# RozDavid/UnScene3D

Hardware: AMD Instinct MI355X
Metric: training scenes/sec (Res16UNet34C+Mask3D, 150k voxels) (higher is better)
Workload: dtype f32

## Files before the change

include/usc3d.h:

```cpp
#ifndef USC3D_H
#define USC3D_H

#include <stdint.h>

#ifdef __cplusplus
extern "C" {
#endif

typedef void* usc_stream_t;

enum usc_status {
  USC_OK = 0,
  USC_ERR_ARG = -1,
  USC_ERR_LAUNCH = -2,
  USC_ERR_RANGE = -3
};

const char* usc_last_error(void);
int usc_abi_version(void);
const char* usc_build_info(void);
int usc_device_count(void);


int usc_voxel_floor_f64(const double* xyz, int64_t n, double voxel_size,
// ... 261 lines not shown
                         float* invstd, float* scale, float* shift, void* ws,
                         int64_t ws_bytes, usc_stream_t s);
int usc_bn_apply(const float* x, const float* scale, const float* shift,
                 const float* residual, int32_t relu, float* y, int64_t n,
                 int32_t c, usc_stream_t s);
int usc_bn_backward_dx(const float* x, const float* dy, const float* y_out,
                       const float* mean, const float* invstd,
                       const float* gamma, const float* mean_g,
                       const float* mean_gxhat, float* dx, float* dres,
                       int64_t n, int32_t c, usc_stream_t s);
int64_t usc_bn_tile_max_rows(void);
int64_t usc_bn_plan(int64_t n, int32_t c, int32_t backward);
int usc_bn_tile_ok(int64_t n, int32_t c);
int64_t usc_bn_tile_ws_bytes(int32_t c);
int usc_bn_tile_forward(const float* partial, int32_t G, float* y, int64_t n,
                        int32_t c, const float* gamma, const float* beta,
                        float eps, float momentum, float* running_mean,
                        float* running_var, int64_t* num_batches_tracked,
                        float* mean, float* invstd, float* scale, float* shift,
                        const float* residual, int32_t relu, float* out,
                        void* ws, int64_t ws_bytes, usc_stream_t s);
int usc_bn_tile_backward(const float* partial, int32_t G, int32_t accumulate,
                         float* dout, const float* y, const float* y_out,
                         const float* mean, const float* invstd,
                         const float* gamma, int64_t n, int32_t c,
                         int32_t training, int32_t dbn_accumulate,
                         float* dgamma, float* dbeta, float* dy, float* dres,
                         void* ws, int64_t ws_bytes, usc_stream_t s);
int usc_bn_backward_reduce(const float* x, const float* dy, const float* y_out,
                           const float* mean, const float* invstd, int64_t n,
                           int32_t c, int32_t training, int32_t accumulate, float* dgamma,
                           float* dbeta, float* mean_g, float* mean_gxhat,
                           void* ws, int64_t ws_bytes, usc_stream_t s);
int usc_relu_fwd(const float* x, float* y, int64_t numel, usc_stream_t s);
int usc_relu_bwd(const float* y, const float* dy, float* dx, int64_t numel,
                 usc_stream_t s);

int usc_avgpool_down2(const float* in, int32_t c, const int32_t* nbr2,
                      int64_t n_coarse, float* out, usc_stream_t s);
int usc_avgpool_down2_ex(const float* in, int32_t c, int32_t ld,
                         const int64_t* row_of, const int32_t* nbr2,
                         int64_t n_coarse, float* out, uint8_t* mask_out,
                         usc_stream_t s);

int usc_gather_rows(const float* src, int32_t c, const int64_t* idx, int64_t n,
                    float* out, usc_stream_t s);

int usc_scatter_add_rows(const float* src, int32_t c, const int64_t* idx,
                         int64_t n, float* dst, usc_stream_t s);

int usc_scatter_rows_unique(const float* src, int32_t c, const int64_t* idx,
                            int64_t n, float* dst, usc_stream_t s);
int usc_scatter_rows_unique_add(const float* src, int32_t c, const int64_t* idx,
                                int64_t n, float* dst, usc_stream_t s);

int64_t usc_sample_keys_ws_bytes(int32_t n_scenes, int32_t K, int32_t q);
int usc_sample_keys(const float* feats, int32_t c, const uint8_t* mask, int32_t q, const float* pos, int32_t p,
                    const int64_t* idx, int32_t n_scenes, int32_t K, const int32_t* n_valid, float* out_feats,
                    uint8_t* out_mask, float* out_pos, void* ws, int64_t ws_bytes, usc_stream_t s);

int64_t usc_attn_mask_rows_ws_bytes(int32_t n_scenes, int32_t K, int32_t q, int32_t d);
int usc_attn_mask_rows(const float* in, int32_t ld, int32_t q, int32_t d, const int32_t* const* tabs,
                       const int64_t* n_rows, const int64_t* idx, int32_t n_scenes, int32_t K,
                       const int32_t* n_valid, uint8_t* out_mask, void* ws, int64_t ws_bytes, int32_t skip_fix,
                       usc_stream_t s);

// ... 373 lines not shown
```

unscene3d_amd/_lib.py:

```python
from __future__ import annotations

import ctypes as C
import os

import torch

_HERE = os.path.dirname(os.path.abspath(__file__))
LIB_PATH = os.environ.get("USC3D_LIB") or os.path.join(_HERE, "libusc3d_hip.so")

_p = C.c_void_p
_i32 = C.c_int32
_i64 = C.c_int64
_f64 = C.c_double
_f32 = C.c_float

class KMap(C.Structure):
    _fields_ = [("nbr", _p), ("perm", _p), ("tile_mask", _p), ("pair_in", _p), ("pair_out", _p), ("koff", _p),
                ("n_in", _i64), ("n_out", _i64), ("pair_capacity", _i64), ("K", _i32), ("reserved", _i32)]


class BNDesc(C.Structure):
    _fields_ = [("gamma", _p), ("beta", _p), ("running_mean", _p), ("running_var", _p), ("num_batches_tracked", _p),
                ("eps", _f32), ("momentum", _f32), ("c", _i32), ("training", _i32)]

# ... 71 lines not shown
    "usc_spconv_wgrad_group_max": (_i32, []),
    "usc_spconv_wgrad_grid_limit": (None, [_i32]),
    "usc_spconv_wgrad_group_ok": (C.c_int, [_i32, _i32, _i32, _i32, _i64]),
    "usc_spconv_wgrad_group": (C.c_int, [_i32, _p, _p, _p, _i32, _i32, _i32, _p, _p, _p, _i64, _i32, _p]),
    "usc_spconv_wgrad_table_ws_bytes": (_i64, [_i32, _i32, _i32]),
    "usc_spconv_wgrad_table": (C.c_int, [_p, _i32, _p, _i32, _p, _i32, _i64, _p, _i32, _p, _i64, _p]),
    "usc_set_wgrad_lane": (C.c_int, [_p, _p, _i64, _i64]),
    "usc_wgrad_lane_join": (C.c_int, [_p]),
    "usc_wgrad_lane_hold": (C.c_int, [_i32, _i64, _i64, _p]),
    "usc_wgrad_lane_holding": (_i32, []),
    "usc_launch_stats_begin": (C.c_int, [_p, _i64, _p]),
    "usc_launch_stats_end": (_i64, [_p, _i64]),
    "usc_wall_clock_khz": (_i64, []),
    "usc_conv_ws_bytes": (_i64, [_kp, _i32, _i32, _i32]),
    "usc_unit_ws_bytes": (_i64, [_kp, _i32, _i32, _i32]),
    "usc_conv_forward": (C.c_int, [_kp, _i32, _p, _i32, _p, _i32, _p, _p, _p, _i64, _p]),
    "usc_conv_backward": (C.c_int, [_kp, _i32, _p, _i32, _p, _i32, _p, _p, _i32, _p, _i32, _p, _i64, _p]),
    "usc_bn_eval_stats": (C.c_int, [_p, _p, _p, _p, _f32, _i32, _p, _p, _p, _p, _p]),
    "usc_conv_bn_act_forward": (C.c_int, [_kp, _i32, _p, _i32, _p, _i32, _bp, _p, _i32, _p, _p, _p, _p, _i64, _p]),
    "usc_unit_bf16_ws_bytes": (_i64, [_kp, _i32, _i32, _i32]),
    "usc_conv_bn_act_forward_bf16": (C.c_int, [_kp, _i32, _p, _i32, _p, _i32, _bp, _p, _i32, _p, _p, _p, _p, _i64, _p]),
    "usc_unit_split_ws_bytes": (_i64, [_kp, _i32, _i32, _i32, _i32]),
    "usc_conv_bn_act_forward_split": (C.c_int, [_kp, _i32, _p, _i32, _p, _i32, _i32, _bp, _p, _i32, _p, _p, _p, _p, _i64, _p]),
    "usc_conv_bn_act_backward_split": (C.c_int, [_kp, _i32, _p, _i32, _p, _i32, _i32, _bp, _p, _p, _p, _p, _p, _p, _p, _i32, _p,
                                                 _i32, _p, _p, _i32, _p, _i64, _p]),
    "usc_conv_bn_act_backward": (C.c_int, [_kp, _i32, _p, _i32, _p, _i32, _bp, _p, _p, _p, _p, _p, _p, _p, _i32, _p,
                                           _i32, _p, _p, _i32, _p, _i64, _p]),
    "usc_colstats_ws_bytes": (_i64, [_i64, _i32]),
    "usc_colstats": (C.c_int, [_p, _p, _i64, _i32, _p, _p, _p, _i64, _p]),
    "usc_bn_apply": (C.c_int, [_p, _p, _p, _p, _i32, _p, _i64, _i32, _p]),
    "usc_bn_backward_dx": (C.c_int, [_p, _p, _p, _p, _p, _p, _p, _p, _p, _p, _i64, _i32, _p]),
    "usc_bn_backward_reduce": (C.c_int, [_p, _p, _p, _p, _p, _i64, _i32, _i32, _i32, _p, _p, _p, _p, _p, _i64, _p]),
    "usc_bn_forward_stats": (C.c_int, [_p, _i64, _i32, _p, _p, _f32, _f32, _p, _p, _p, _p, _p, _p, _p, _p, _i64, _p]),
    "usc_relu_fwd": (C.c_int, [_p, _p, _i64, _p]),
    "usc_relu_bwd": (C.c_int, [_p, _p, _p, _i64, _p]),
    "usc_avgpool_down2": (C.c_int, [_p, _i32, _p, _i64, _p, _p]),
    "usc_avgpool_down2_ex": (C.c_int, [_p, _i32, _i32, _p, _p, _i64, _p, _p, _p]),
    "usc_gather_rows": (C.c_int, [_p, _i32, _p, _i64, _p, _p]),
    "usc_scatter_add_rows": (C.c_int, [_p, _i32, _p, _i64, _p, _p]),
    "usc_scatter_rows_unique": (C.c_int, [_p, _i32, _p, _i64, _p, _p]),
    "usc_scatter_rows_unique_add": (C.c_int, [_p, _i32, _p, _i64, _p, _p]),
    "usc_sample_keys_ws_bytes": (_i64, [_i32, _i32, _i32]),
    "usc_sample_keys": (C.c_int, [_p, _i32, _p, _i32, _p, _i32, _p, _i32, _i32, _p, _p, _p, _p, _p, _i64, _p]),
    "usc_attn_mask_rows_ws_bytes": (_i64, [_i32, _i32, _i32, _i32]),
    "usc_attn_mask_rows": (C.c_int, [_p, _i32, _i32, _i32, _p, _p, _p, _i32, _i32, _p, _p, _p, _i64, _i32, _p]),
    "usc_segment_csr_ws_bytes": (_i64, [_i64, _i64]),
    "usc_segment_csr": (C.c_int, [_p, _i64, _i64, _p, _p, _p, _i64, _p]),
    "usc_segment_mean_fwd": (C.c_int, [_p, _i32, _p, _p, _i64, _p, _p]),
    "usc_segment_mean_bwd": (C.c_int, [_p, _i32, _p, _p, _i64, _p, _p]),
    "usc_segment_mean_nonzero": (C.c_int, [_p, _i32, _p, _p, _i64, _p, _p, _p]),
    "usc_segment_max_nonzero": (C.c_int, [_p, _i32, _p, _p, _i64, _p, _p, _p]),
    "usc_ncut_similarity": (C.c_int, [_p, _i64, _i32, _i32, _p, _p, _p]),
    "usc_ncut_similarity_masked": (C.c_int, [_p, _p, _i64, _i32, _i32, _p, _p, _p]),
    "usc_ncut_normalize_mat": (C.c_int, [_p, _i64, _p, _i64, _p]),
    "usc_ncut_binarize": (C.c_int, [_p, _p, _i64, _f32, _f64, _p, _p, _p, _p]),
    "usc_ncut_fiedler_ws_bytes": (_i64, [_i64]),
    "usc_ncut_fiedler": (C.c_int, [_p, _p, _i64, _f64, _p, _p, _p, _i64, _p]),
    "usc_ncut_fiedler_ex": (C.c_int, [_p, _p, _i64, _f64, _p, _p, _p, _i64, _p, _i32]),
    "usc_ncut_fiedler_plan": (_i32, [_i64, _i32, _i32]),
    "usc_knn1": (C.c_int, [_p, _i64, _p, _i64, _p, _p, _p]),
    "usc_knn1_grid_ws_bytes": (_i64, [_i64, _p]),
    "usc_knn1_grid": (C.c_int, [_p, _i64, _p, _i64, _p, _f64, _p, _p, _p, _p, _i64, _p]),
    "usc_knn_hybrid_grid_ws_bytes": (_i64, [_i64, _p]),
    "usc_knn_hybrid_grid": (C.c_int, [_p, _i64, _p, _i64, _f32, _i32, _p, _f64, _p, _p, _p, _p, _i64, _p]),
    "usc_normals_pca": (C.c_int, [_p, _i64, _p, _i64, _p, _p, _i32, _p, _p]),
    "usc_cc_eps_init": (C.c_int, [_p, _i64, _p]),
# ... 148 lines not shown
```

unscene3d_amd/csrc/rows.hip:

```cpp
#include <math.h>
#include <stdlib.h>

#include "common.h"
#include "scan.h"

namespace usc {

void launch_group_reduce(const float* partial, int G, int64_t numel4, int cout, const float* bias, int accumulate,
                         float* out, hipStream_t st);

enum StatMode { STAT_XY = 0, STAT_BN_BWD = 1 };

struct StatArgs {
  const float* x;
  const float* y;
  const float* y_out;
  const float* mean;
  const float* invstd;
  int64_t n;
  int c;
};

constexpr int kStatMaxBlocks = 1024;
constexpr int kStatUnroll = 4;

template <int VEC, int MODE>
__global__ __launch_bounds__(256) void colstats_kernel(StatArgs a, double* __restrict__ partial) {
  extern __shared__ double sh[];
  const int c = a.c;
  const int CT = c / VEC;
  const int RP = 256 / CT;
  const int rl = threadIdx.x / CT, cg = threadIdx.x - rl * CT;
  const bool active = rl < RP;
  double s1[VEC], s2[VEC];
#pragma unroll
  for (int v = 0; v < VEC; ++v) s1[v] = s2[v] = 0.0;
  float mu[VEC], is[VEC];
  if (MODE == STAT_BN_BWD && active) {
#pragma unroll
    for (int v = 0; v < VEC; ++v) {
      mu[v] = a.mean[cg * VEC + v];
      is[v] = a.invstd[cg * VEC + v];
    }
  }
  if (active) {
    const int64_t stride = (int64_t)gridDim.x * RP;
    for (int64_t r0 = (int64_t)blockIdx.x * RP + rl; r0 < a.n; r0 += stride * kStatUnroll) {
      float xv[kStatUnroll][VEC], yv[kStatUnroll][VEC], ov[kStatUnroll][VEC];
#pragma unroll
      for (int u = 0; u < kStatUnroll; ++u) {
        const int64_t r = r0 + u * stride;
        if (r < a.n) {
          const int64_t off = r * c + cg * VEC;
          if (VEC == 4) {
            float4 t = *reinterpret_cast<const float4*>(a.x + off);
            xv[u][0] = t.x; xv[u][1] = t.y; xv[u][2] = t.z; xv[u][3] = t.w;
            if (a.y) {
              float4 w = *reinterpret_cast<const float4*>(a.y + off);
              yv[u][0] = w.x; yv[u][1] = w.y; yv[u][2] = w.z; yv[u][3] = w.w;
            }
            if (MODE == STAT_BN_BWD && a.y_out) {
              float4 w = *reinterpret_cast<const float4*>(a.y_out + off);
              ov[u][0] = w.x; ov[u][1] = w.y; ov[u][2] = w.z; ov[u][3] = w.w;
            }
          } else {
            xv[u][0] = a.x[off];
            if (a.y) yv[u][0] = a.y[off];
            if (MODE == STAT_BN_BWD && a.y_out) ov[u][0] = a.y_out[off];
          }
        }
      }
#pragma unroll
      for (int u = 0; u < kStatUnroll; ++u) {
        if (r0 + u * stride < a.n) {
#pragma unroll
          for (int v = 0; v < VEC; ++v) {
            if (MODE == STAT_XY) {
              s1[v] += (double)xv[u][v];
              s2[v] += (double)xv[u][v] * (double)(a.y ? yv[u][v] : xv[u][v]);
            } else {
              float g = yv[u][v];
              if (a.y_out && !(ov[u][v] > 0.f)) g = 0.f;
              const float xhat = (xv[u][v] - mu[v]) * is[v];
              s1[v] += (double)g;
              s2[v] += (double)g * (double)xhat;
            }
          }
        }
      }
    }
#pragma unroll
    for (int v = 0; v < VEC; ++v) {
      sh[((int64_t)rl * c + cg * VEC + v) * 2 + 0] = s1[v];
      sh[((int64_t)rl * c + cg * VEC + v) * 2 + 1] = s2[v];
    }
  }
  __syncthreads();
  for (int ch = threadIdx.x; ch < c; ch += 256) {
    double t1 = 0.0, t2 = 0.0;
    for (int r = 0; r < RP; ++r) {
      t1 += sh[((int64_t)r * c + ch) * 2 + 0];
// ... 157 lines not shown
    }
  }
}

__global__ void bn_eval_stats_kernel(const float* __restrict__ gamma, const float* __restrict__ beta,
                                     const float* __restrict__ rmean, const float* __restrict__ rvar, float eps, int c,
                                     float* __restrict__ mean, float* __restrict__ invstd, float* __restrict__ scale,
                                     float* __restrict__ shift) {
  const int ch = blockIdx.x * blockDim.x + threadIdx.x;
  if (ch >= c) return;
  const float is = 1.f / sqrtf(rvar[ch] + eps);
  const float sc = gamma[ch] * is;
  mean[ch] = rmean[ch];
  invstd[ch] = is;
  scale[ch] = sc;
  shift[ch] = beta[ch] - rmean[ch] * sc;
}

static int colstats_vec(int c) {
  if (c < 1 || c > 1024) return 0;
  const int vec = (c % 4 == 0 && c / 4 <= 256) ? 4 : 1;
  return c / vec <= 256 ? vec : 0;
}
static int colstats_blocks(int64_t n, int c, int vec) {
  const int CT = c / vec, RP = 256 / CT;
  int64_t b = ceil_div(n, (int64_t)RP * 4 * kStatUnroll);
  if (b > kStatMaxBlocks) b = kStatMaxBlocks;
  if (b < 1) b = 1;
  return (int)b;
}

template <int MODE>
static int launch_colstats_partials(const StatArgs& a, void* ws, int64_t ws_bytes, hipStream_t st, const char* name,
                                    int* nblocks_out) {
  const int c = a.c;
  const int vec = colstats_vec(c);
  USC_REQUIRE(vec > 0, "%s: unsupported channel count %d", name, c);
  const int nb = colstats_blocks(a.n, c, vec);
  USC_REQUIRE(ws_bytes >= (int64_t)nb * 2 * c * 8, "%s: workspace too small", name);
  const int RP = 256 / (c / vec);
  const size_t lds = (size_t)RP * c * 2 * sizeof(double);
  double* partial = (double*)ws;
  if (vec == 4)
    hipLaunchKernelGGL((colstats_kernel<4, MODE>), dim3(nb), dim3(256), lds, st, a, partial);
  else
    hipLaunchKernelGGL((colstats_kernel<1, MODE>), dim3(nb), dim3(256), lds, st, a, partial);
  *nblocks_out = nb;
  return USC_OK;
}

constexpr int kSampleRows = 16;
constexpr int kSampleMaxQ = 256;
constexpr int kSampleMaxScenes = 16;
struct SampleArgs {
  const float* feats; const unsigned char* mask; const float* pos; const int64_t* idx;
  float* out_feats; unsigned char* out_mask; float* out_pos; unsigned char* part;
  int c, q, p, K, nblk, qs;
  int n_valid[kSampleMaxScenes];
};

template <int NQ>
__global__ __launch_bounds__(256) void sample_keys_kernel(SampleArgs a) {
  __shared__ unsigned char acc[4][128 * NQ];
  const int lane = threadIdx.x & 63, wave = threadIdx.x >> 6;
  const int b = blockIdx.y, k0 = blockIdx.x * kSampleRows + wave * 4;
  const int c4 = a.c >> 2, p4 = a.p >> 2;
  const int nvalid = a.n_valid[b];
  const bool has_pos = a.pos != nullptr;
  int64_t src[4];
#pragma unroll
  for (int r = 0; r < 4; ++r) {
    const int k = k0 + r < a.K ? k0 + r : a.K - 1;
    src[r] = a.idx[(int64_t)b * a.K + k];
  }
  float4 f0[4], f1[4], q0[4], q1[4];
  unsigned char ma[4], mb[4], mc[NQ > 1 ? 4 : 1], md[NQ > 1 ? 4 : 1];
  const bool fa = lane < c4, fb = lane + 64 < c4, pa = has_pos && lane < p4, pb = has_pos && lane + 64 < p4;
  const bool qa = lane < a.q, qb = lane + 64 < a.q, qc = NQ > 1 && lane + 128 < a.q, qd = NQ > 1 && lane + 192 < a.q;
#pragma unroll
// ... 906 lines not shown
    const float4 mx = *reinterpret_cast<const float4*>(tile_sh + c + ch0);
    const float ga0 = a.gamma[ch0], ga1 = a.gamma[ch0 + 1], ga2 = a.gamma[ch0 + 2], ga3 = a.gamma[ch0 + 3];
    float4 o;
    o.x = ga0 * is.x * (gv.x - mg.x - (xv.x - mu.x) * is.x * mx.x);
    o.y = ga1 * is.y * (gv.y - mg.y - (xv.y - mu.y) * is.y * mx.y);
    o.z = ga2 * is.z * (gv.z - mg.z - (xv.z - mu.z) * is.z * mx.z);
    o.w = ga3 * is.w * (gv.w - mg.w - (xv.w - mu.w) * is.w * mx.w);
    *reinterpret_cast<float4*>(a.dx + e) = o;
  }
}

struct BnTileGeom { int tr, ntiles, ncb; };
static BnTileGeom bn_tile_geom(int64_t n, int c) {
  BnTileGeom g;
  const int64_t per = ceil_div(n, (int64_t)kBnTileMaxTiles);
  g.tr = (int)(ceil_div(per, (int64_t)kBnTileRowLanes) * kBnTileRowLanes);
  g.ntiles = (int)ceil_div(n, (int64_t)g.tr);
  g.ncb = c / 32;
  return g;
}
static int bn_apply_grid(int64_t nvec) {
  int64_t g = ceil_div(nvec, (int64_t)256 * 2);
  if (g > 1024) g = 1024;
  if (g < 1) g = 1;
  return (int)g;
}

static bool tile_form_on() {
  static const bool on = usc_bn_tile_max_rows() > 0;
  return on;
}
bool tile_rows_ok(int64_t n, int c) { return tile_form_on() && n <= usc_bn_tile_max_rows() && usc_bn_tile_ok(n, c); }

}

using namespace usc;

extern "C" {

int64_t usc_bn_plan(int64_t n, int32_t c, int32_t backward) {
  USC_REQUIRE(n >= 1 && c >= 1, "usc_bn_plan: bad sizes");
  int64_t code = 0;
  if (bn_small_ok(n, c, backward != 0)) {
    code = 1 | ((int64_t)bn_small_remap(c / 4) << 2);
  } else if (const int vec = colstats_vec(c)) {
    code = 2 | ((int64_t)vec << 3) | ((int64_t)colstats_blocks(n, c, vec) << 8);
  }
  if (usc_bn_tile_ok(n, c)) {
    const BnTileGeom g = bn_tile_geom(n, c);
    code |= ((int64_t)1 << 20) | ((int64_t)g.ntiles << 24) | ((int64_t)g.tr << 32);
  }
  if (tile_rows_ok(n, c)) code |= (int64_t)1 << 21;
  return code;
}

int64_t usc_colstats_ws_bytes(int64_t n, int32_t c) { (void)n; return (int64_t)kStatMaxBlocks * 2 * c * 8; }

int usc_colstats(const float* x, const float* y, int64_t n, int32_t c, double* sum1, double* sum2, void* ws,
                 int64_t ws_bytes, usc_stream_t s) {
  USC_REQUIRE(x && sum1 && sum2 && ws && n >= 0, "usc_colstats: bad argument");
  StatArgs a{x, y, nullptr, nullptr, nullptr, n, (int)c};
  int nb = 0;
  int rc = launch_colstats_partials<STAT_XY>(a, ws, ws_bytes, as_stream(s), "usc_colstats", &nb);
  if (rc) return rc;
  hipLaunchKernelGGL(colstats_final_kernel, dim3((unsigned)c), dim3(64), 0, as_stream(s), (const double*)ws, nb, (int)c,
                     sum1, sum2);
// ... 21 lines not shown
  USC_CHECK_LAUNCH("usc_bn_forward_stats");
  return USC_OK;
}

int usc_bn_eval_stats(const float* gamma, const float* beta, const float* running_mean, const float* running_var, float eps,
                      int32_t c, float* mean, float* invstd, float* scale, float* shift, usc_stream_t s) {
  USC_REQUIRE(gamma && beta && running_mean && running_var && mean && invstd && scale && shift && c >= 1,
              "usc_bn_eval_stats: bad argument");
  hipLaunchKernelGGL(bn_eval_stats_kernel, dim3((unsigned)ceil_div(c, 256)), dim3(256), 0, as_stream(s), gamma, beta,
                     running_mean, running_var, eps, (int)c, mean, invstd, scale, shift);
  USC_CHECK_LAUNCH("usc_bn_eval_stats");
  return USC_OK;
}

int usc_bn_backward_reduce(const float* x, const float* dy, const float* y_out, const float* mean, const float* invstd,
                           int64_t n, int32_t c, int32_t training, int32_t accumulate, float* dgamma, float* dbeta,
                           float* mean_g, float* mean_gxhat, void* ws, int64_t ws_bytes, usc_stream_t s) {
  USC_REQUIRE(x && dy && mean && invstd && dgamma && dbeta && mean_g && mean_gxhat && ws && n >= 1,
              "usc_bn_backward_reduce: bad argument");
  StatArgs a{x, dy, y_out, mean, invstd, n, (int)c};
  BnBwdOut o{dgamma, dbeta, mean_g, mean_gxhat, n, (int)training, (int)accumulate};
  if (bn_small_ok(n, c, true)) {
    hipLaunchKernelGGL((bn_small_kernel<STAT_BN_BWD, BnBwdOut>), dim3((unsigned)(c / 4)), dim3(256), 0, as_stream(s), a, o);
    USC_CHECK_LAUNCH("usc_bn_backward_reduce");
    return USC_OK;
  }
  int nb = 0;
  int rc = launch_colstats_partials<STAT_BN_BWD>(a, ws, ws_bytes, as_stream(s), "usc_bn_backward_reduce", &nb);
  if (rc) return rc;
  hipLaunchKernelGGL(bn_bwd_finalize_kernel, dim3((unsigned)c), dim3(64), 0, as_stream(s), (const double*)ws, nb, (int)c, o);
  USC_CHECK_LAUNCH("usc_bn_backward_reduce");
  return USC_OK;
}

int usc_bn_apply(const float* x, const float* scale, const float* shift, const float* residual, int32_t relu, float* y,
                 int64_t n, int32_t c, usc_stream_t s) {
  USC_REQUIRE(n >= 0 && c >= 1, "usc_bn_apply: bad sizes");
  if (n == 0) return USC_OK;
  USC_REQUIRE(x && scale && shift && y, "usc_bn_apply: null pointer");
  const int64_t numel = n * c;
  if (c % 4 == 0)
    hipLaunchKernelGGL((bn_apply_kernel<4>), dim3(stream_grid(numel / 4, 256)), dim3(256), 0, as_stream(s), x, scale,
                       shift, residual, (int)relu, y, numel / 4, (int)c);
  else
    hipLaunchKernelGGL((bn_apply_kernel<1>), dim3(stream_grid(numel, 256)), dim3(256), 0, as_stream(s), x, scale,
                       shift, residual, (int)relu, y, numel, (int)c);
  USC_CHECK_LAUNCH("usc_bn_apply");
  return USC_OK;
}

int usc_bn_backward_dx(const float* x, const float* dy, const float* y_out, const float* mean, const float* invstd,
                       const float* gamma, const float* mean_g, const float* mean_gxhat, float* dx, float* dres,
                       int64_t n, int32_t c, usc_stream_t s) {
  USC_REQUIRE(n >= 0 && c >= 1, "usc_bn_backward_dx: bad sizes");
  if (n == 0) return USC_OK;
  USC_REQUIRE(x && dy && mean && invstd && gamma && mean_g && mean_gxhat && dx, "usc_bn_backward_dx: null pointer");
  const int64_t numel = n * c;
  if (c % 4 == 0)
    hipLaunchKernelGGL((bn_bwd_dx_kernel<4>), dim3(stream_grid(numel / 4, 256)), dim3(256), 0, as_stream(s), x, dy,
                       y_out, mean, invstd, gamma, mean_g, mean_gxhat, dx, dres, numel / 4, (int)c);
  else
    hipLaunchKernelGGL((bn_bwd_dx_kernel<1>), dim3(stream_grid(numel, 256)), dim3(256), 0, as_stream(s), x, dy, y_out,
                       mean, invstd, gamma, mean_g, mean_gxhat, dx, dres, numel, (int)c);
  USC_CHECK_LAUNCH("usc_bn_backward_dx");
  return USC_OK;
}
// ... 376 lines not shown
```

unscene3d_amd/csrc/units.hip:

```cpp
#include <stdlib.h>

#include <vector>

#include "common.h"

namespace usc { bool tile_rows_ok(int64_t n, int c); }

using namespace usc;

namespace {

struct WsCursor {
  char* base; int64_t bytes; int64_t off;
  void* take(int64_t n) {
    n = align_up(n > 0 ? n : 16, 256);
    if (off + n > bytes) return nullptr;
    void* p = base + off;
    off += n;
    return p;
  }
  int64_t left() const { return bytes - off; }
  void* rest() { return base + off; }
};

inline bool table_is_compact(int64_t n_out, int cin, int cout, int K) {
  return (usc_spconv_plan(0, n_out, cin, cout, K) >> 12) & 1;
}
inline bool sorted_ok(const usc_kmap* m, int cin, int cout) {
  return m->nbr && m->perm && m->tile_mask && m->K > 1 && m->K <= 32 && cin % 32 == 0 && cout % 32 == 0 && cin <= 4096;
}

struct TableGemmPlan {
  bool sorted;
  int64_t wt_bytes;
  int64_t gemm_bytes;
};
TableGemmPlan plan_table_gemm(const usc_kmap* m, int64_t n_out, int cin, int cout, int K, bool wt) {
  const bool compact = m->nbr && table_is_compact(n_out, cin, cout, K);
  if (sorted_ok(m, cin, cout) && !compact) return {true, 0, usc_spconv_sorted_ws_bytes(n_out, cin, cout, K)};
// ... 248 lines not shown

int conv_backward_impl(const usc_kmap* m, int32_t kind, const float* x, int32_t cin, const float* W, int32_t cout,
                       const float* dy, float* dx, int32_t dx_accumulate, float* dW, int32_t dW_accumulate, void* ws,
                       int64_t ws_bytes, usc_stream_t s, Pending* out, int planes = 0) {
  if (out) *out = Pending{};
  int rc = check_map(m, kind, cin, cout, "usc_conv_backward");
  if (rc) return rc;
  const ConvShape sh = conv_shape(m, kind);
  const int K = m->K;
  USC_REQUIRE(x && W && dy, "usc_conv_backward: null pointer");
  WsCursor cur{(char*)ws, ws ? ws_bytes : 0, 0};
  WgradJob job = wgrad_job(m, kind, sh, x, dy, dW, cin, cout);
  if (dW && dW_accumulate && x && dy) {
    Lane* lane = lane_for_current_device();
    const bool lane_ok = lane && sh.n_in > 0 && sh.n_in <= lane->max_rows && sh.n_out <= lane->max_rows &&
                         job.list_bytes <= lane->ws_bytes && (!m->nbr || (m->pair_in && m->pair_out && m->koff));
    const int64_t big = sh.n_in > sh.n_out ? sh.n_in : sh.n_out;
    if (lane && lane->hold && big <= lane->release_max_rows) { rc = lane_release(lane, s); if (rc) return rc; }
    if (lane_ok && lane->hold && big >= lane->hold_min_rows) {
      job.nbr = nullptr;
      lane->held.push_back(job);
      dW = nullptr;
    } else if (lane_ok &&
        hipEventRecord(lane->fork, as_stream(s)) == hipSuccess && hipStreamWaitEvent(lane->st, lane->fork, 0) == hipSuccess) {
      lane->dirty = true;
      rc = issue_wgrad(job, 1, lane->ws, lane->ws_bytes, (usc_stream_t)lane->st);
      if (rc) return rc;
      dW = nullptr;
    }
  }
  int64_t dgrad_bytes = 0;
  Slices left;
  const bool split_dx = planes > 0 && kind == USC_CONV_SAME && split_dgrad_ok(m, cin, cout, planes);
  const bool may_defer = !split_dx && out && dx && tile_rows_ok(sh.n_in, cin);
  if (may_defer) {
    int64_t f_, w_;
    conv_ws_parts(m, kind, cin, cout, &f_, &dgrad_bytes, &w_);
    if (dgrad_bytes + w_ > cur.bytes) dgrad_bytes = 0;
  }
  Slices* want = (may_defer && dgrad_bytes > 0) ? &left : nullptr;
  if (dx && sh.n_in > 0) {
    if (split_dx) {
      rc = planes_gemm(m, planes, dy, sh.n_out, cout, W, nullptr, cin, sh.n_in, 1, false, dx, dx_accumulate, cur, s,
                       "usc_conv_backward");
    } else if (kind == USC_CONV_SAME) {
      rc = table_gemm(m, dy, sh.n_out, cout, W, K, cin, sh.n_in, nullptr, dx, dx_accumulate, 1, cur, s, want);
    } else {
      const bool down = kind == USC_CONV_DOWN;
      USC_REQUIRE(!down || !dx_accumulate, "usc_conv_backward: accumulate is not supported on the pair-list form");
      USC_REQUIRE(!down || (m->pair_in && m->pair_out && m->koff), "usc_conv_backward: strided conv needs the pair lists");
      float* Wt = (float*)cur.take((int64_t)K * cin * cout * 4);
      USC_REQUIRE(Wt, "usc_conv_backward: workspace too small");
      rc = usc_weight_transpose(W, K, cin, cout, 0, Wt, s);
      if (!rc) rc = down ? usc_spconv_pairs_gemm(dy, cout, Wt, K, cin, m->pair_out, m->pair_in, m->koff, sh.n_in, dx, s)
                         : table_gemm(m, dy, sh.n_out, cout, Wt, K, cin, sh.n_in, nullptr, dx, dx_accumulate, 0, cur, s, want);
    }
    if (!rc && left.G > 0) {
      out->dx = dx; out->partial = left.partial; out->G = left.G; out->n = sh.n_in; out->c = cin; out->accumulate = dx_accumulate;
    }
    if (rc) dW = nullptr;
  }
  if (dW) {
    WsCursor wc{(char*)ws, ws ? ws_bytes : 0, left.G > 0 ? dgrad_bytes : 0};
    void* w = wc.take(job.list_bytes);
    if (!w) { set_error("usc_conv_backward: workspace too small (weight gradient)"); return USC_ERR_ARG; }
    rc = issue_wgrad(job, dW_accumulate, w, (char*)ws + ws_bytes - (char*)w, s);
  }
  return rc;
}

bool bn_tile_form(const usc_bn* bn, int64_t n, int c, int64_t sb) {
  return bn->training && tile_rows_ok(n, c) && sb >= usc_bn_tile_ws_bytes(c);
}

int bn_act_tail(const char* who, const usc_bn* bn, bool tile, Slices left, float* y, int64_t n, int cout,
                const float* residual, int relu, float* stats, float* out, void* sws, int64_t sb, usc_stream_t s) {
  float* mean = stats, *invstd = stats + cout, *scale = stats + 2 * cout, *shift = stats + 3 * cout;
  if (tile)
    return usc_bn_tile_forward(left.partial, left.G, y, n, cout, bn->gamma, bn->beta, bn->eps, bn->momentum, bn->running_mean,
                               bn->running_var, bn->num_batches_tracked, mean, invstd, scale, shift, residual, relu, out, sws,
                               sb, s);
  int rc;
  if (bn->training) {
    rc = usc_bn_forward_stats(y, n, cout, bn->gamma, bn->beta, bn->eps, bn->momentum, bn->running_mean, bn->running_var,
                              bn->num_batches_tracked, mean, invstd, scale, shift, sws, sb, s);
  } else {
    USC_REQUIRE(bn->running_mean && bn->running_var, "%s: eval mode needs running statistics", who);
    rc = usc_bn_eval_stats(bn->gamma, bn->beta, bn->running_mean, bn->running_var, bn->eps, cout, mean, invstd, scale,
                           shift, s);
  }
  if (rc) return rc;
  return usc_bn_apply(y, scale, shift, residual, relu, out, n, cout, s);
}

struct FwdForm {
  const char* who;
  const char* map_who;
  const char* ws_note;
  int P;
};
int forward_unit(const FwdForm& f, const usc_kmap* m, int32_t kind, const float* x, int32_t cin, const float* W,
                 const uint16_t* Wp, int32_t cout, const usc_bn* bn, const float* residual, int32_t relu, float* y,
                 float* stats, float* out, void* ws, int64_t ws_bytes, usc_stream_t s) {
  int rc = check_map(m, kind, cin, cout, f.map_who);
  if (rc) return rc;
  USC_REQUIRE(bn && bn->c == cout, "%s: batch-norm width must equal the conv's output width", f.who);
  USC_REQUIRE(y && stats && out && bn->gamma && bn->beta, "%s: null pointer", f.who);
  const ConvShape sh = conv_shape(m, kind);
  if (f.P) {
    const int64_t gb = f.P == 1 ? usc_spconv_gather_gemm_bf16_ws_bytes(sh.n_out, cin, cout, m->K)
                                : usc_spconv_gather_gemm_split_ws_bytes(sh.n_out, cin, cout, m->K, f.P);
    USC_REQUIRE(gb >= 0, "%s: shape not covered (K=%d, %d -> %d channels)", f.who, m->K, cin, cout);
  }
  if (sh.n_out == 0) return USC_OK;
  if (f.P) {
    USC_REQUIRE(x && (f.P == 1 ? (const void*)Wp : (const void*)W), "%s: null pointer", f.who);
    USC_REQUIRE(m->nbr || kind == USC_CONV_SAME, "%s: strided maps need the child table", f.who);
  }
  WsCursor cur{(char*)ws, ws ? ws_bytes : 0, 0};
  const int64_t sb = usc_colstats_ws_bytes(sh.n_out, cout);
  void* sws = cur.take(sb);
  USC_REQUIRE(sws, "%s: workspace too small%s", f.who, f.ws_note);
  const bool tile = f.P != 1 && bn_tile_form(bn, sh.n_out, cout, sb);
  Slices left;
  if (f.P == 0) rc = conv_forward_impl(m, kind, x, cin, W, cout, nullptr, y, cur.rest(), cur.left(), s, tile ? &left : nullptr);
  else rc = planes_gemm(m, f.P, x, sh.n_in, cin, W, Wp, cout, sh.n_out, 0, kind == USC_CONV_UP, y, 0, cur, s, f.who);
  if (rc) return rc;
  return bn_act_tail(f.who, bn, tile, left, y, sh.n_out, cout, residual, relu, stats, out, sws, sb, s);
}

int unit_backward_impl(const usc_kmap* m, int32_t kind, const float* x, int32_t cin, const float* W, int32_t cout,
                       const usc_bn* bn, const float* y, const float* stats, const float* out_relu,
                       const float* dout, float* dy, float* dres, float* dx, int32_t dx_accumulate, float* dW,
                       int32_t dW_accumulate, float* dgamma, float* dbeta, int32_t dbn_accumulate, void* ws,
                       int64_t ws_bytes, usc_stream_t s, Pending* in, Pending* out, int planes = 0) {
  if (out) *out = Pending{};
  USC_REQUIRE(bn && bn->c == cout, "usc_conv_bn_act_backward: batch-norm width must equal the conv's output width");
  USC_REQUIRE(y && stats && dout && dy && dgamma && dbeta && bn->gamma, "usc_conv_bn_act_backward: null pointer");
  const ConvShape sh = conv_shape(m, kind);
  if (sh.n_out == 0) return USC_OK;
  if (planes > 0)
    USC_REQUIRE(ws && ws_bytes >= usc_unit_split_ws_bytes(m, kind, cin, cout, planes),
                "usc_conv_bn_act_backward_split: workspace too small (usc_unit_split_ws_bytes)");
  WsCursor cur{(char*)ws, ws ? ws_bytes : 0, 0};
  const int64_t sb = usc_colstats_ws_bytes(sh.n_out, cout);
  void* sws = cur.take(sb);
  float* red = (float*)cur.take(2 * (int64_t)cout * 4);
  USC_REQUIRE(sws && red, "usc_conv_bn_act_backward: workspace too small");
  const float* mean = stats, *invstd = stats + cout;
  int rc;
  const bool has_in = in && in->G > 0;
  if (has_in) USC_REQUIRE(in->dx == dout && in->n == sh.n_out && in->c == cout, "usc unit: pending slices do not belong to this unit");
  if (tile_rows_ok(sh.n_out, cout) && sb >= usc_bn_tile_ws_bytes(cout)) {
    rc = usc_bn_tile_backward(has_in ? in->partial : nullptr, has_in ? in->G : 0, has_in ? in->accumulate : 0, (float*)dout, y,
                              out_relu, mean, invstd, bn->gamma, sh.n_out, cout, bn->training, dbn_accumulate, dgamma,
                              dbeta, dy, dres, sws, sb, s);
    if (has_in) *in = Pending{};
    if (rc) return rc;
  } else {
    if (has_in) { rc = flush_pending(*in, s); if (rc) return rc; }
    rc = usc_bn_backward_reduce(y, dout, out_relu, mean, invstd, sh.n_out, cout, bn->training, dbn_accumulate, dgamma,
                                dbeta, red, red + cout, sws, sb, s);
    if (rc) return rc;
    rc = usc_bn_backward_dx(y, dout, out_relu, mean, invstd, bn->gamma, red, red + cout, dy, dres, sh.n_out, cout, s);
    if (rc) return rc;
  }
  return conv_backward_impl(m, kind, x, cin, W, cout, dy, dx, dx_accumulate, dW, dW_accumulate, cur.rest(), cur.left(), s, out,
                            planes);
}

int check_split(const usc_kmap* m, int32_t kind, int32_t P, const char* who) {
  USC_REQUIRE(m, "%s: null kernel map", who);
  USC_REQUIRE(P == 2 || P == 3, "%s: P must be 2 or 3 (got %d)", who, P);
  USC_REQUIRE(kind == USC_CONV_SAME, "%s: the split precision covers stride-1 units only", who);
  return USC_OK;
}

int64_t program_half_bytes(const usc_step* steps, int32_t n_steps) {
  int64_t need = 256;
  if (!steps) return need;
  for (int i = 0; i < n_steps; ++i) {
    const usc_step& t = steps[i];
    if ((t.op == USC_STEP_UNIT_FWD || t.op == USC_STEP_UNIT_BWD) && t.map) {
      int64_t b = usc_unit_ws_bytes(t.map, t.kind, t.cin, t.cout);
      if (t.split_planes) {
        const int64_t sb = usc_unit_split_ws_bytes(t.map, t.kind, t.cin, t.cout, t.split_planes);
        if (sb > b) b = sb;
      }
      if (b > need) need = b;
    } else if (t.op == USC_STEP_UNIT_FWD_BF16 && t.map) {
      const int64_t b = usc_unit_bf16_ws_bytes(t.map, t.kind, t.cin, t.cout);
      if (b > need) need = b;
    }
  }
  return align_up(need, 256);
// ... 302 lines not shown
```

Measured before the change: 46.73.

## Fuse split-K partial slice reduction into BN statistics kernels for large maps

For maps too large for the tile form, the conv's G partial output slices are now summed inside the batch-norm column-statistics kernel. The kernel writes the reduced rows and accumulates their statistics in the same pass, in both forward and backward. Previously the slices were reduced by a separate group-reduce or flush kernel before the stats kernel. This saves one full read and write of the activation and a launch, at the cost of more registers per thread (a batch of nine float4 loads per unroll) and an env-gated heuristic that limits G to 5 or fewer.

```diff
diff --git a/include/usc3d.h b/include/usc3d.h
--- a/include/usc3d.h
+++ b/include/usc3d.h
@@ -317,6 +317,21 @@
                            int32_t c, int32_t training, int32_t accumulate, float* dgamma,
                            float* dbeta, float* mean_g, float* mean_gxhat,
                            void* ws, int64_t ws_bytes, usc_stream_t s);
+int usc_bn_forward_stats_slices(const float* partial, int32_t G, float* y, int64_t n,
+                                int32_t c, const float* gamma, const float* beta,
+                                float eps, float momentum, float* running_mean,
+                                float* running_var, int64_t* num_batches_tracked,
+                                float* mean, float* invstd, float* scale, float* shift,
+                                void* ws, int64_t ws_bytes, usc_stream_t s);
+int usc_bn_backward_reduce_slices(const float* partial, int32_t G, int32_t accumulate,
+                                  float* dout, const float* y, const float* y_out,
+                                  const float* mean, const float* invstd, int64_t n,
+                                  int32_t c, int32_t training, int32_t dbn_accumulate,
+                                  float* dgamma, float* dbeta, float* mean_g,
+                                  float* mean_gxhat, void* ws, int64_t ws_bytes,
+                                  usc_stream_t s);
+int32_t usc_bn_slices_ok(int64_t n, int32_t c, int32_t G);
+int64_t usc_bn_slices_calls(int32_t backward);
 int usc_relu_fwd(const float* x, float* y, int64_t numel, usc_stream_t s);
 int usc_relu_bwd(const float* y, const float* dy, float* dx, int64_t numel,
                  usc_stream_t s);
diff --git a/unscene3d_amd/_lib.py b/unscene3d_amd/_lib.py
--- a/unscene3d_amd/_lib.py
+++ b/unscene3d_amd/_lib.py
@@ -127,6 +127,12 @@
     "usc_bn_backward_dx": (C.c_int, [_p, _p, _p, _p, _p, _p, _p, _p, _p, _p, _i64, _i32, _p]),
     "usc_bn_backward_reduce": (C.c_int, [_p, _p, _p, _p, _p, _i64, _i32, _i32, _i32, _p, _p, _p, _p, _p, _i64, _p]),
     "usc_bn_forward_stats": (C.c_int, [_p, _i64, _i32, _p, _p, _f32, _f32, _p, _p, _p, _p, _p, _p, _p, _p, _i64, _p]),
+    "usc_bn_forward_stats_slices": (C.c_int, [_p, _i32, _p, _i64, _i32, _p, _p, _f32, _f32, _p, _p, _p, _p, _p, _p, _p, _p, _i64,
+                                              _p]),
+    "usc_bn_backward_reduce_slices": (C.c_int, [_p, _i32, _i32, _p, _p, _p, _p, _p, _i64, _i32, _i32, _i32, _p, _p, _p, _p, _p,
+                                                _i64, _p]),
+    "usc_bn_slices_ok": (_i32, [_i64, _i32, _i32]),
+    "usc_bn_slices_calls": (_i64, [_i32]),
     "usc_relu_fwd": (C.c_int, [_p, _p, _i64, _p]),
     "usc_relu_bwd": (C.c_int, [_p, _p, _p, _i64, _p]),
     "usc_avgpool_down2": (C.c_int, [_p, _i32, _p, _i64, _p, _p]),
diff --git a/unscene3d_amd/csrc/rows.hip b/unscene3d_amd/csrc/rows.hip
--- a/unscene3d_amd/csrc/rows.hip
+++ b/unscene3d_amd/csrc/rows.hip
@@ -1,5 +1,7 @@
 #include <math.h>
 #include <stdlib.h>
+
+#include <atomic>
 
 #include "common.h"
 #include "scan.h"
@@ -24,8 +26,17 @@
 constexpr int kStatMaxBlocks = 1024;
 constexpr int kStatUnroll = 4;
 
-template <int VEC, int MODE>
-__global__ __launch_bounds__(256) void colstats_kernel(StatArgs a, double* __restrict__ partial) {
+struct StatSlices {
+  const float* partial;
+  int G;
+  int64_t slice;
+  float* dst;
+  int accumulate;
+};
+constexpr int kSliceBatch = 9;
+
+template <int VEC, int MODE, bool SLICES = false>
+__global__ __launch_bounds__(256) void colstats_kernel(StatArgs a, double* __restrict__ partial, StatSlices sl) {
   extern __shared__ double sh[];
   const int c = a.c;
   const int CT = c / VEC;
@@ -52,7 +63,16 @@
         const int64_t r = r0 + u * stride;
         if (r < a.n) {
           const int64_t off = r * c + cg * VEC;
-          if (VEC == 4) {
+          if (SLICES && VEC == 4) {
+            if (MODE == STAT_BN_BWD) {
+              float4 t = *reinterpret_cast<const float4*>(a.x + off);
+              xv[u][0] = t.x; xv[u][1] = t.y; xv[u][2] = t.z; xv[u][3] = t.w;
+              if (a.y_out) {
+                float4 w = *reinterpret_cast<const float4*>(a.y_out + off);
+                ov[u][0] = w.x; ov[u][1] = w.y; ov[u][2] = w.z; ov[u][3] = w.w;
+              }
+            }
+          } else if (VEC == 4) {
             float4 t = *reinterpret_cast<const float4*>(a.x + off);
             xv[u][0] = t.x; xv[u][1] = t.y; xv[u][2] = t.z; xv[u][3] = t.w;
             if (a.y) {
@@ -67,6 +87,49 @@
             xv[u][0] = a.x[off];
             if (a.y) yv[u][0] = a.y[off];
             if (MODE == STAT_BN_BWD && a.y_out) ov[u][0] = a.y_out[off];
+          }
+        }
+      }
+      if (SLICES && VEC == 4) {
+        float4 acc[kStatUnroll];
+#pragma unroll
+        for (int u = 0; u < kStatUnroll; ++u) {
+          const int64_t r = r0 + u * stride;
+          acc[u] = make_float4(0.f, 0.f, 0.f, 0.f);
+          if (MODE == STAT_BN_BWD && sl.accumulate && r < a.n) acc[u] = *reinterpret_cast<const float4*>(sl.dst + r * c + cg * VEC);
+        }
+        for (int g0 = 0; g0 < sl.G; g0 += kSliceBatch) {
+          float4 t[kStatUnroll][kSliceBatch];
+#pragma unroll
+          for (int j = 0; j < kSliceBatch; ++j) {
+            if (g0 + j < sl.G) {
+              const float* pp = sl.partial + (int64_t)(g0 + j) * sl.slice + cg * VEC;
+#pragma unroll
+              for (int u = 0; u < kStatUnroll; ++u) {
+                const int64_t r = r0 + u * stride;
+                if (r < a.n) t[u][j] = *reinterpret_cast<const float4*>(pp + r * c);
+              }
+            }
+          }
+#pragma unroll
+          for (int j = 0; j < kSliceBatch; ++j) {
+            if (g0 + j < sl.G) {
+#pragma unroll
+              for (int u = 0; u < kStatUnroll; ++u) {
+                if (r0 + u * stride < a.n) {
+                  acc[u].x += t[u][j].x; acc[u].y += t[u][j].y; acc[u].z += t[u][j].z; acc[u].w += t[u][j].w;
+                }
+              }
+            }
+          }
+        }
+#pragma unroll
+        for (int u = 0; u < kStatUnroll; ++u) {
+          const int64_t r = r0 + u * stride;
+          if (r < a.n) {
+            *reinterpret_cast<float4*>(sl.dst + r * c + cg * VEC) = acc[u];
+            float* into = MODE == STAT_XY ? xv[u] : yv[u];
+            into[0] = acc[u].x; into[1] = acc[u].y; into[2] = acc[u].z; into[3] = acc[u].w;
           }
         }
       }
@@ -290,19 +353,22 @@
 
 template <int MODE>
 static int launch_colstats_partials(const StatArgs& a, void* ws, int64_t ws_bytes, hipStream_t st, const char* name,
-                                    int* nblocks_out) {
+                                    int* nblocks_out, const StatSlices* sl = nullptr) {
   const int c = a.c;
   const int vec = colstats_vec(c);
   USC_REQUIRE(vec > 0, "%s: unsupported channel count %d", name, c);
+  USC_REQUIRE(!sl || vec == 4, "%s: the slices form needs a channel count that is a multiple of 4 (got %d)", name, c);
   const int nb = colstats_blocks(a.n, c, vec);
   USC_REQUIRE(ws_bytes >= (int64_t)nb * 2 * c * 8, "%s: workspace too small", name);
   const int RP = 256 / (c / vec);
   const size_t lds = (size_t)RP * c * 2 * sizeof(double);
   double* partial = (double*)ws;
-  if (vec == 4)
-    hipLaunchKernelGGL((colstats_kernel<4, MODE>), dim3(nb), dim3(256), lds, st, a, partial);
+  if (sl)
+    hipLaunchKernelGGL((colstats_kernel<4, MODE, true>), dim3(nb), dim3(256), lds, st, a, partial, *sl);
+  else if (vec == 4)
+    hipLaunchKernelGGL((colstats_kernel<4, MODE>), dim3(nb), dim3(256), lds, st, a, partial, StatSlices{});
   else
-    hipLaunchKernelGGL((colstats_kernel<1, MODE>), dim3(nb), dim3(256), lds, st, a, partial);
+    hipLaunchKernelGGL((colstats_kernel<1, MODE>), dim3(nb), dim3(256), lds, st, a, partial, StatSlices{});
   *nblocks_out = nb;
   return USC_OK;
 }
@@ -1275,6 +1341,18 @@
 }
 bool tile_rows_ok(int64_t n, int c) { return tile_form_on() && n <= usc_bn_tile_max_rows() && usc_bn_tile_ok(n, c); }
 
+static int slices_form_mode() {
+  static const int mode = [] { const char* e = getenv("USC3D_BN_SLICES"); return e && e[0] == '0' ? 0 : e && e[0] == '2' ? 2 : 1; }();
+  return mode;
+}
+bool slices_rows_ok(int64_t n, int c, bool backward) {
+  return slices_form_mode() > 0 && !tile_rows_ok(n, c) && colstats_vec(c) == 4 && !bn_small_ok(n, c, backward);
+}
+bool slices_form_ok(int64_t n, int c, int G, bool backward) {
+  return G >= 1 && slices_rows_ok(n, c, backward) && (slices_form_mode() == 2 || usc_bn_slices_ok(n, c, G));
+}
+static std::atomic<int64_t> g_slices_calls[2];
+
 }
 
 using namespace usc;
@@ -1362,6 +1440,56 @@
   USC_CHECK_LAUNCH("usc_bn_backward_reduce");
   return USC_OK;
 }
+
+int usc_bn_forward_stats_slices(const float* partial, int32_t G, float* y, int64_t n, int32_t c, const float* gamma,
+                                const float* beta, float eps, float momentum, float* running_mean, float* running_var,
+                                int64_t* num_batches_tracked, float* mean, float* invstd, float* scale, float* shift,
+                                void* ws, int64_t ws_bytes, usc_stream_t s) {
+  const char* who = "usc_bn_forward_stats_slices";
+  USC_REQUIRE(partial && G >= 1 && y && gamma && beta && mean && invstd && scale && shift && ws && n >= 1, "%s: bad argument", who);
+  USC_REQUIRE((running_mean == nullptr) == (running_var == nullptr), "%s: running stats mismatch", who);
+  USC_REQUIRE(c >= 4 && c % 4 == 0, "%s: the channel count must be a multiple of 4 (got %d)", who, (int)c);
+  USC_REQUIRE(!bn_small_ok(n, c, false), "%s: maps of up to %lld rows are not served (the tile form's range)", who,
+              (long long)bn_small_rows(false));
+  StatArgs a{nullptr, nullptr, nullptr, nullptr, nullptr, n, (int)c};
+  StatSlices sl{partial, (int)G, n * c, y, 0};
+  BnFwdOut o{gamma, beta, running_mean, running_var, mean, invstd, scale, shift, eps, momentum, n, num_batches_tracked};
+  int nb = 0;
+  int rc = launch_colstats_partials<STAT_XY>(a, ws, ws_bytes, as_stream(s), who, &nb, &sl);
+  if (rc) return rc;
+  hipLaunchKernelGGL(bn_fwd_finalize_kernel, dim3((unsigned)c), dim3(64), 0, as_stream(s), (const double*)ws, nb, (int)c, o);
+  USC_CHECK_LAUNCH(who);
+  ++g_slices_calls[0];
+  return USC_OK;
+}
+
+int usc_bn_backward_reduce_slices(const float* partial, int32_t G, int32_t accumulate, float* dout, const float* y,
+                                  const float* y_out, const float* mean, const float* invstd, int64_t n, int32_t c,
+                                  int32_t training, int32_t dbn_accumulate, float* dgamma, float* dbeta, float* mean_g,
+                                  float* mean_gxhat, void* ws, int64_t ws_bytes, usc_stream_t s) {
+  const char* who = "usc_bn_backward_reduce_slices";
+  USC_REQUIRE(partial && G >= 1 && dout && y && mean && invstd && dgamma && dbeta && mean_g && mean_gxhat && ws && n >= 1,
+              "%s: bad argument", who);
+  USC_REQUIRE(c >= 4 && c % 4 == 0, "%s: the channel count must be a multiple of 4 (got %d)", who, (int)c);
+  USC_REQUIRE(!bn_small_ok(n, c, true), "%s: maps of up to %lld rows are not served (the tile form's range)", who,
+              (long long)bn_small_rows(true));
+  StatArgs a{y, dout, y_out, mean, invstd, n, (int)c};
+  StatSlices sl{partial, (int)G, n * c, dout, (int)(accumulate != 0)};
+  BnBwdOut o{dgamma, dbeta, mean_g, mean_gxhat, n, (int)training, (int)dbn_accumulate};
+  int nb = 0;
+  int rc = launch_colstats_partials<STAT_BN_BWD>(a, ws, ws_bytes, as_stream(s), who, &nb, &sl);
+  if (rc) return rc;
+  hipLaunchKernelGGL(bn_bwd_finalize_kernel, dim3((unsigned)c), dim3(64), 0, as_stream(s), (const double*)ws, nb, (int)c, o);
+  USC_CHECK_LAUNCH(who);
+  ++g_slices_calls[1];
+  return USC_OK;
+}
+
+int32_t usc_bn_slices_ok(int64_t n, int32_t c, int32_t G) {
+  return n >= 1 && c >= 4 && c % 4 == 0 && c <= 1024 && G >= 1 && G <= 5;
+}
+
+int64_t usc_bn_slices_calls(int32_t backward) { return g_slices_calls[backward ? 1 : 0].load(); }
 
 int usc_bn_apply(const float* x, const float* scale, const float* shift, const float* residual, int32_t relu, float* y,
                  int64_t n, int32_t c, usc_stream_t s) {
diff --git a/unscene3d_amd/csrc/units.hip b/unscene3d_amd/csrc/units.hip
--- a/unscene3d_amd/csrc/units.hip
+++ b/unscene3d_amd/csrc/units.hip
@@ -4,7 +4,11 @@
 
 #include "common.h"
 
-namespace usc { bool tile_rows_ok(int64_t n, int c); }
+namespace usc {
+bool tile_rows_ok(int64_t n, int c);
+bool slices_rows_ok(int64_t n, int c, bool backward);
+bool slices_form_ok(int64_t n, int c, int G, bool backward);
+}
 
 using namespace usc;
 
@@ -319,7 +323,7 @@
   int64_t dgrad_bytes = 0;
   Slices left;
   const bool split_dx = planes > 0 && kind == USC_CONV_SAME && split_dgrad_ok(m, cin, cout, planes);
-  const bool may_defer = !split_dx && out && dx && tile_rows_ok(sh.n_in, cin);
+  const bool may_defer = !split_dx && out && dx && (tile_rows_ok(sh.n_in, cin) || slices_rows_ok(sh.n_in, cin, true));
   if (may_defer) {
     int64_t f_, w_;
     conv_ws_parts(m, kind, cin, cout, &f_, &dgrad_bytes, &w_);
@@ -368,6 +372,17 @@
                                bn->running_var, bn->num_batches_tracked, mean, invstd, scale, shift, residual, relu, out, sws,
                                sb, s);
   int rc;
+  if (left.G > 0 && bn->training && slices_form_ok(n, cout, left.G, false)) {
+    rc = usc_bn_forward_stats_slices(left.partial, left.G, y, n, cout, bn->gamma, bn->beta, bn->eps, bn->momentum,
+                                     bn->running_mean, bn->running_var, bn->num_batches_tracked, mean, invstd, scale, shift,
+                                     sws, sb, s);
+    if (rc) return rc;
+    return usc_bn_apply(y, scale, shift, residual, relu, out, n, cout, s);
+  }
+  if (left.G > 0) {
+    rc = usc_group_reduce(left.partial, left.G, n, cout, nullptr, 0, y, s);
+    if (rc) return rc;
+  }
   if (bn->training) {
     rc = usc_bn_forward_stats(y, n, cout, bn->gamma, bn->beta, bn->eps, bn->momentum, bn->running_mean, bn->running_var,
                               bn->num_batches_tracked, mean, invstd, scale, shift, sws, sb, s);
@@ -409,8 +424,9 @@
   void* sws = cur.take(sb);
   USC_REQUIRE(sws, "%s: workspace too small%s", f.who, f.ws_note);
   const bool tile = f.P != 1 && bn_tile_form(bn, sh.n_out, cout, sb);
+  const bool slices = !tile && f.P == 0 && bn->training && cout % 4 == 0 && slices_rows_ok(sh.n_out, cout, false);
   Slices left;
-  if (f.P == 0) rc = conv_forward_impl(m, kind, x, cin, W, cout, nullptr, y, cur.rest(), cur.left(), s, tile ? &left : nullptr);
+  if (f.P == 0) rc = conv_forward_impl(m, kind, x, cin, W, cout, nullptr, y, cur.rest(), cur.left(), s, tile || slices ? &left : nullptr);
   else rc = planes_gemm(m, f.P, x, sh.n_in, cin, W, Wp, cout, sh.n_out, 0, kind == USC_CONV_UP, y, 0, cur, s, f.who);
   if (rc) return rc;
   return bn_act_tail(f.who, bn, tile, left, y, sh.n_out, cout, residual, relu, stats, out, sws, sb, s);
@@ -445,9 +461,15 @@
     if (has_in) *in = Pending{};
     if (rc) return rc;
   } else {
-    if (has_in) { rc = flush_pending(*in, s); if (rc) return rc; }
-    rc = usc_bn_backward_reduce(y, dout, out_relu, mean, invstd, sh.n_out, cout, bn->training, dbn_accumulate, dgamma,
-                                dbeta, red, red + cout, sws, sb, s);
+    if (has_in && slices_form_ok(sh.n_out, cout, in->G, true)) {
+      rc = usc_bn_backward_reduce_slices(in->partial, in->G, in->accumulate, (float*)dout, y, out_relu, mean, invstd, sh.n_out,
+                                         cout, bn->training, dbn_accumulate, dgamma, dbeta, red, red + cout, sws, sb, s);
+      *in = Pending{};
+    } else {
+      if (has_in) { rc = flush_pending(*in, s); if (rc) return rc; }
+      rc = usc_bn_backward_reduce(y, dout, out_relu, mean, invstd, sh.n_out, cout, bn->training, dbn_accumulate, dgamma,
+                                  dbeta, red, red + cout, sws, sb, s);
+    }
     if (rc) return rc;
     rc = usc_bn_backward_dx(y, dout, out_relu, mean, invstd, bn->gamma, red, red + cout, dy, dres, sh.n_out, cout, s);
     if (rc) return rc;
```

Result: no change. 46.59 (-0.3%).
